# SFXiang/ORB-SLAM2-Annotation

Measured on AMD Instinct MI355X. Metric: frames/sec ORB extract+match (1000 feat, 640×480 mono) at 1/2/4/8 GPU; % HBM roofline, higher is better.
Workload: dtype u8

## Files before the change

### orb-slam2-annotation_amd/csrc/describe.hip

```cpp
#include "orbgpu_internal.h"
#include "orbgpu_kernels.h"
#include "blur_device.h"
#include "group_sum.h"
#include "../../include/orbgpu.h"

#include <algorithm>
#include <cstddef>
#include <cstdlib>
#include <type_traits>

namespace orbgpu {

namespace {

constexpr signed char kPattern[1024] = {
#include "bit_pattern_31.inc"
};
struct PatternF { float4 t[256]; };
constexpr PatternF make_pattern_f() {
    PatternF p{};
    for (int i = 0; i < 256; ++i)
        p.t[i] = float4{(float)kPattern[4 * i], (float)kPattern[4 * i + 2], (float)kPattern[4 * i + 1],
                        (float)kPattern[4 * i + 3]};
    return p;
}
__constant__ PatternF c_pattern = make_pattern_f();

constexpr int kUmax[16] = {15, 15, 15, 15, 14, 14, 14, 13, 13, 12, 11, 10, 9, 8, 6, 3};

#ifndef ORBGPU_DESC_RPITCH
#define ORBGPU_DESC_RPITCH 48
#endif
constexpr int kRPitchC = ORBGPU_DESC_RPITCH;
constexpr int kRWidth = 48;
static_assert(kRPitchC % 4 == 0 && kRPitchC >= kRWidth, "raw pitch");
constexpr int kDiscWords = 31 * 9, kDiscLoads = (kDiscWords + 63) / 64;
struct DiscWord { uint32_t m1, mc, mv, off; };
struct DiscLut { DiscWord w[4][kDiscLoads * 64]; };
constexpr DiscLut make_disc_lut() {
    DiscLut L{};
    for (int od = 0; od < 4; ++od)
        for (int idx = 0; idx < kDiscWords; ++idx) {
            const int r = idx / 9, q = idx % 9, v = r - 15, d = kUmax[v < 0 ? -v : v];
            DiscWord e{0u, 0u, 0u, (uint32_t)(r * kRPitchC + 4 * q)};
            for (int b = 0; b < 4; ++b) {
                const int u = 4 * q + b - od - 15;
                if (u >= -d && u <= d) {
                    e.m1 |= 1u << (8 * b);
                    e.mc |= (uint32_t)(4 * q + b) << (8 * b);
                    e.mv |= (uint32_t)(v + 15) << (8 * b);
                }
            }
            L.w[od][idx] = e;
        }
    return L;
}
__constant__ DiscLut c_disc = make_disc_lut();
struct DiscTail { DiscWord w[4][64]; };
constexpr DiscTail make_disc_tail() {
    DiscTail T{};
    const DiscLut L = make_disc_lut();
    for (int od = 0; od < 4; ++od)
        for (int i = 0; i < 64; ++i) T.w[od][i] = L.w[od][256 + i];
    return T;
}
__constant__ DiscTail c_disc_tail = make_disc_tail();
static_assert(kDiscLoads == 5, "the disc loads are four from c_disc and one from c_disc_tail");

__device__ inline float fast_atan2(float y, float x) {
    const float k = (float)(180 / M_PI);
    const float p1 = 0.9997878412794807f * k, p3 = -0.3258083974640975f * k;
    const float p5 = 0.1555786518463281f * k, p7 = -0.04432655554792128f * k;
    const float ax = fabsf(x), ay = fabsf(y);
    const float eps = (float)2.220446049250313080847e-16;
    float a, c, c2;
    if (ax >= ay) {
        c = __fdiv_rn(ay, __fadd_rn(ax, eps));
        c2 = __fmul_rn(c, c);
        a = __fmul_rn(__fadd_rn(__fmul_rn(__fadd_rn(__fmul_rn(__fadd_rn(__fmul_rn(p7, c2), p5), c2), p3), c2), p1), c);
    } else {
        c = __fdiv_rn(ax, __fadd_rn(ay, eps));
        c2 = __fmul_rn(c, c);
        a = __fsub_rn(90.f, __fmul_rn(__fadd_rn(__fmul_rn(__fadd_rn(__fmul_rn(__fadd_rn(__fmul_rn(p7, c2), p5), c2), p3), c2), p1), c));
    }
    if (x < 0) a = __fsub_rn(180.f, a);
    if (y < 0) a = __fsub_rn(360.f, a);
    return a;
}

struct SinCosTab { double sign[4], hpi_inv, hpi, c0, c1, c2, c3, c4, s1, s2, s3; };
__constant__ SinCosTab c_sc[2] = {
    {{1.0, -1.0, -1.0, 1.0}, 0x1.45F306DC9C883p+23, 0x1.921FB54442D18p0, 0x1p0, -0x1.ffffffd0c621cp-2,
     0x1.55553e1068f19p-5, -0x1.6c087e89a359dp-10, 0x1.99343027bf8c3p-16, -0x1.555545995a603p-3,
     0x1.1107605230bc4p-7, -0x1.994eb3774cf24p-13},
    {{1.0, -1.0, -1.0, 1.0}, 0x1.45F306DC9C883p+23, 0x1.921FB54442D18p0, -0x1p0, 0x1.ffffffd0c621cp-2,
     -0x1.55553e1068f19p-5, 0x1.6c087e89a359dp-10, -0x1.99343027bf8c3p-16, -0x1.555545995a603p-3,
     0x1.1107605230bc4p-7, -0x1.994eb3774cf24p-13}};

__device__ inline uint32_t top12(float x) { return (__float_as_uint(x) >> 20) & 0x7ff; }

__device__ inline float sc_poly(double x, double x2, const SinCosTab* p, int n) {
    if ((n & 1) == 0) {
        const double x3 = __dmul_rn(x, x2);
        const double s1 = __fma_rn(x2, p->s3, p->s2);
        const double x7 = __dmul_rn(x3, x2);
        const double s = __fma_rn(x3, p->s1, x);
        return __double2float_rn(__fma_rn(x7, s1, s));
    }
    const double x4 = __dmul_rn(x2, x2);
    const double c2 = __fma_rn(x2, p->c4, p->c3);
    const double c1 = __fma_rn(x2, p->c1, p->c0);
    const double x6 = __dmul_rn(x4, x2);
    const double c = __fma_rn(x4, p->c2, c1);
    return __double2float_rn(__fma_rn(x6, c2, c));
}

__device__ inline void glibc_sincosf(float y, float* sinp, float* cosp) {
    double x = y;
    if (top12(y) < top12(0x1.921FB6p-1f)) {
        if (top12(y) < top12(0x1p-12f)) { *sinp = y; *cosp = 1.0f; return; }
        const double x2 = __dmul_rn(x, x);
        *sinp = sc_poly(x, x2, &c_sc[0], 0);
        *cosp = sc_poly(x, x2, &c_sc[0], 1);
        return;
    }
    const double r = __dmul_rn(x, c_sc[0].hpi_inv);
    const int n = ((int32_t)r + 0x800000) >> 24;
    x = __fma_rn(-(double)n, c_sc[0].hpi, x);
    const double s = c_sc[0].sign[n & 3];
    const SinCosTab* p = (n & 2) ? &c_sc[1] : &c_sc[0];
    const double xs = __dmul_rn(x, s), x2 = __dmul_rn(x, x);
    *sinp = sc_poly(xs, x2, p, n);
    *cosp = sc_poly(xs, x2, p, n ^ 1);
}

__device__ inline uint32_t wave_total(uint32_t v) {
    v += (uint32_t)__builtin_amdgcn_update_dpp(0, (int)v, kDppXor1, 0xF, 0xF, true);
    v += (uint32_t)__builtin_amdgcn_update_dpp(0, (int)v, kDppXor2, 0xF, 0xF, true);
    v += (uint32_t)__builtin_amdgcn_update_dpp(0, (int)v, kDppHalfMirror, 0xF, 0xF, true);
    v += (uint32_t)__builtin_amdgcn_update_dpp(0, (int)v, kDppMirror, 0xF, 0xF, true);
    v += (uint32_t)__builtin_amdgcn_update_dpp(0, (int)v, 0x142, 0xA, 0xF, false);
    v += (uint32_t)__builtin_amdgcn_update_dpp(0, (int)v, 0x143, 0xC, 0xF, false);
    return (uint32_t)__builtin_amdgcn_readlane((int)v, 63);
}

constexpr int kBPitch = 40;
constexpr int kRPitch = kRPitchC;
constexpr int kRawWords = kPatch * (kRWidth / 4);
constexpr int kQuads = kBPitch / 4;
constexpr int kColChunks = (kBlur + 6) / 7;

__device__ inline void wave_sync() {
    asm volatile("s_waitcnt lgkmcnt(0)" ::: "memory");
    __builtin_amdgcn_wave_barrier();
}

__device__ inline int reflect101(int p, int n) { return p < 0 ? -p : (p >= n ? 2 * n - 2 - p : p); }

#ifndef ORBGPU_DESC_KEYS
#define ORBGPU_DESC_KEYS 1
#endif
constexpr int kKeysPerWave = ORBGPU_DESC_KEYS;

#ifndef DESC_LDS_PROBE
#define DESC_LDS_PROBE 0
#endif
static_assert(kKeysPerWave == 1 || kKeysPerWave == 2 || kKeysPerWave == 4, "ORBGPU_DESC_KEYS: 1, 2 or 4");

constexpr int kRawBytes = (kPatch * kRPitch + 15) & ~15;
constexpr int kBlurSlotBytes = (kBlur * kBPitch + 15) & ~15;
struct alignas(16) DescLds {
    uint8_t raw[kRawBytes];
    uint8_t blur[kKeysPerWave][kBlurSlotBytes];
};
static_assert(offsetof(DescLds, blur) % 16 == 0 && kBlurSlotBytes % 16 == 0, "16-byte dump stores into blur[k]");

#ifndef ORBGPU_DESC_SCALAR_COUNTS
#define ORBGPU_DESC_SCALAR_COUNTS 1
#endif

struct KeyRef {
    int l, i, before, cx, cy;
    uint32_t key;
};

__device__ bool key_ref(const Geom& g, int f, int slot, int lane, const uint32_t* __restrict__ oct_out,
                        const int* __restrict__ oct_count, int* __restrict__ counts, KeyRef& K) {
    uint32_t se = g.slot_tab[slot];
    uint32_t key = oct_out[(size_t)f * g.slots_frame + slot];
#if ORBGPU_DESC_SCALAR_COUNTS
    (void)lane;
    se = (uint32_t)__builtin_amdgcn_readfirstlane((int)se);
    key = (uint32_t)__builtin_amdgcn_readfirstlane((int)key);
    const int l = (int)(se & 15u), i = (int)(se >> 4);
    const int* cr = oct_count + (size_t)f * kOcStride;
    int cv[kMaxLevels];
#pragma unroll
    for (int j = 0; j < kMaxLevels; ++j) cv[j] = cr[j];
    int before = 0, mine = 0, total = 0;
#pragma unroll
    for (int j = 0; j < kMaxLevels; ++j) {
        const int cj = j < g.nlevels ? cv[j] : 0;
        before += j < l ? cj : 0;
        mine = j == l ? cj : mine;
        total += cj;
    }
    if (slot == 0 && lane == 0) counts[f] = total;
#else
    const int ll = lane & 15;
    int c = oct_count[(size_t)f * kOcStride + ll];
    se = (uint32_t)__builtin_amdgcn_readfirstlane((int)se);
    key = (uint32_t)__builtin_amdgcn_readfirstlane((int)key);
    asm volatile("" ::"s"(se), "s"(key), "v"(c));
    c = ll < g.nlevels ? c : 0;
    const int l = (int)(se & 15u), i = (int)(se >> 4);
    int sc = c;
    sc += __builtin_amdgcn_update_dpp(0, sc, 0x111, 0xF, 0xF, true);
    sc += __builtin_amdgcn_update_dpp(0, sc, 0x112, 0xF, 0xF, true);
    sc += __builtin_amdgcn_update_dpp(0, sc, 0x114, 0xF, 0xF, true);
    sc += __builtin_amdgcn_update_dpp(0, sc, 0x118, 0xF, 0xF, true);
    const int mine = __builtin_amdgcn_readlane(c, l);
    const int before = __builtin_amdgcn_readlane(sc, l) - mine;
    if (slot == 0 && lane == 0) counts[f] = __builtin_amdgcn_readlane(sc, 15);
#endif
    if (i >= mine) return false;
    K.l = l;
    K.i = i;
    K.before = before;
    K.key = key;
    K.cx = key_x(K.key) + kBorder;
    K.cy = key_y(K.key) + kBorder;
    return true;
}

__device__ int2 describe_patch(const Geom& g, int f, const KeyRef& K, int lane, uint8_t* rawbuf, uint8_t* blur_out,
                               const uint8_t* __restrict__ img0, size_t row0, size_t frame0,
                               const uint8_t* __restrict__ pyr) {
    const int l = K.l, cx = K.cx, cy = K.cy;
    const LevelGeom& L = g.lv[l];
#ifdef DESC_PROBE_SAMEFRAME
    const uint8_t* raw = img0;
    const size_t rp = row0;
    (void)frame0;
#else
    const uint8_t* raw = l == 0 ? img0 + (size_t)f * frame0 : pyr + L.offset + (size_t)f * L.frame_bytes;
    const size_t rp = l == 0 ? row0 : (size_t)L.pitch;
#endif

    const int xb = (cx - kBlurR) & ~3, x0 = xb - 4;
    if (x0 >= 0 && x0 + kRWidth <= L.w && cy - kPatchR >= 0 && cy + kPatchR < L.h) {
        constexpr int kChunks = kPatch * (kRWidth / 16);
        const uint8_t* top = raw + (size_t)(cy - kPatchR) * rp + x0;
        uint4 c[3];
        uint8_t* dst[3];
        uint8_t* const dump = blur_out;
#pragma unroll
        for (int k = 0; k < 3; ++k) {
            const uint32_t idx = (uint32_t)(lane + 64 * k), r = __umul24(idx, 21846u) >> 16, q = idx - 3u * r;
            const uint32_t doff = kRPitch == 48 ? 16u * idx : __umul24(r, (uint32_t)kRPitch) + 16u * q;
            dst[k] = (k < 2 && 64 * 2 <= kChunks) || idx < (uint32_t)kChunks ? rawbuf + doff : dump;
            const uint32_t idxc = k < 2 ? idx : min(idx, (uint32_t)kChunks - 1u), rc = __umul24(idxc, 21846u) >> 16;
            c[k] = load16_a4(top + (uint32_t)(__umul24(rc, (uint32_t)rp - 48u) + 16u * idxc));
        }
#pragma unroll
        for (int k = 0; k < 3; ++k) {
            if constexpr (kRPitch % 16 == 0) {
                *reinterpret_cast<uint4*>(dst[k]) = c[k];
            } else {
                uint32_t* d = reinterpret_cast<uint32_t*>(dst[k]);
                d[0] = c[k].x;
                d[1] = c[k].y;
                d[2] = c[k].z;
                d[3] = c[k].w;
            }
        }
    } else {
    constexpr int kLoads = (kRawWords + 63) / 64;
    uint32_t v[kLoads];
#pragma unroll
    for (int k = 0; k < kLoads; ++k) {
        const int idx = min(lane + 64 * k, kRawWords - 1), r = idx / 12, q = idx - r * 12;
        const uint8_t* row = raw + (size_t)reflect101(cy - kPatchR + r, L.h) * rp;
        const int col = x0 + 4 * q;
        if (col >= 0 && col + 3 < L.w) {
            v[k] = *reinterpret_cast<const uint32_t*>(row + col);
        } else {
            uint32_t w = 0;
            for (int j = 0; j < 4; ++j) w |= (uint32_t)row[reflect101(col + j, L.w)] << (8 * j);
            v[k] = w;
        }
    }
#pragma unroll
    for (int k = 0; k < kLoads; ++k) {
        const int idx = lane + 64 * k, r = idx / 12, q = idx - r * 12;
        if (idx < kRawWords) reinterpret_cast<uint32_t*>(rawbuf)[r * (kRPitch / 4) + q] = v[k];
    }
    }
    wave_sync();

    const int xd = (cx - 15) & ~3, od = cx - 15 - xd;
    const uint8_t* disc = rawbuf + (kPatchR - 15) * kRPitch + (xd - x0);
    uint32_t sp = 0u, cp = 0u, vp = 0u;
    const __attribute__((address_space(1))) uint8_t* dtab =
        (const __attribute__((address_space(1))) uint8_t*)&c_disc.w[od][0];
    const __attribute__((address_space(1))) uint8_t* dtab4 =
        (const __attribute__((address_space(1))) uint8_t*)&c_disc_tail.w[od][0];
#pragma unroll
    for (int k = 0; k < kDiscLoads; ++k) {
        typedef uint32_t u32x4 __attribute__((ext_vector_type(4)));
        const u32x4 t = *(const __attribute__((address_space(1))) u32x4*)((k < 4 ? dtab : dtab4) + 16u * (uint32_t)lane +
                                                                          1024u * (k % 4));
        const DiscWord e{t.x, t.y, t.z, t.w};
#if DESC_LDS_PROBE & 4
        const uint32_t w = *reinterpret_cast<const uint32_t*>(rawbuf + 4 * lane + 256 * k + (e.off & 0));
#else
        const uint32_t w = *reinterpret_cast<const uint32_t*>(disc + e.off);
#endif
        sp = __builtin_amdgcn_udot4(w, e.m1, sp, false);
        cp = __builtin_amdgcn_udot4(w, e.mc, cp, false);
        vp = __builtin_amdgcn_udot4(w, e.mv, vp, false);
    }
    const int m10 = (int)wave_total(cp - __umul24((uint32_t)(od + 15), sp));
    const int m01 = (int)wave_total(vp - __umul24(15u, sp));

    const int simd_end = L.w & ~3;
    auto passes = [&](auto all_simd) {
        const int qq = (int)(__umul24((uint32_t)lane, 10923u) >> 16), c = lane - qq * kColChunks;
        const int q = min(qq, kQuads - 1), r0 = c * 7;
        const bool simd = xb + 4 * q < simd_end, store = qq < kQuads;
#if DESC_LDS_PROBE & 2
        const uint32_t raw0 = 12u * (uint32_t)lane + 0u * (uint32_t)(r0 + q);
#else
        const uint32_t raw0 = __umul24((uint32_t)r0, (uint32_t)kRPitch) + 4u * (uint32_t)q;
#endif
        const uint32_t out0 = __umul24((uint32_t)r0, (uint32_t)kBPitch) + 4u * (uint32_t)q;
        auto row = [&](int k, blurdev::f32x2& lo, blurdev::f32x2& hi) {
            const uint32_t* w = reinterpret_cast<const uint32_t*>(rawbuf + raw0 + k * kRPitch);
            blurdev::Raw3 R3;
            R3.a = w[0];
            R3.b = w[1];
            R3.c = w[2];
            blurdev::row_pass_raw_shifted(R3, lo, hi);
        };
        auto from_next = [](blurdev::f32x2 v) {
            return blurdev::f32x2{
                __int_as_float(__builtin_amdgcn_mov_dpp(__float_as_int(v.x), 0x130, 0xF, 0xF, false)),
                __int_as_float(__builtin_amdgcn_mov_dpp(__float_as_int(v.y), 0x130, 0xF, 0xF, false))};
        };
        blurdev::f32x2 wl[13], wh[13];
#pragma unroll
        for (int k = 0; k < 8; ++k) row(k, wl[k], wh[k]);
#pragma unroll
        for (int j = 0; j < 7; ++j) {
            if (j >= 2) {
                wl[6 + j] = from_next(wl[j - 1]);
                wh[6 + j] = from_next(wh[j - 1]);
            }
            if (store && r0 + j < kBlur) {
                const blurdev::f32x2 lo =
                    blurdev::col_pass(wl[j], wl[j + 1], wl[j + 2], wl[j + 3], wl[j + 4], wl[j + 5], wl[j + 6]);
                const blurdev::f32x2 hi =
                    blurdev::col_pass(wh[j], wh[j + 1], wh[j + 2], wh[j + 3], wh[j + 4], wh[j + 5], wh[j + 6]);
#if DESC_LDS_PROBE & 8
                *reinterpret_cast<uint32_t*>(blur_out + ((4 * lane + 256 * j) & 1023) + (out0 & 0)) =
                    all_simd ? blurdev::pack4_simd(lo, hi) : blurdev::pack4(lo, hi, simd);
#else
                *reinterpret_cast<uint32_t*>(blur_out + out0 + j * kBPitch) =
                    all_simd ? blurdev::pack4_simd(lo, hi) : blurdev::pack4(lo, hi, simd);
#endif
            }
        }
    };
    if (xb + 4 * (kQuads - 1) < simd_end)
        passes(std::true_type{});
    else
        passes(std::false_type{});
    return int2{m10, m01};
}

__device__ void describe_tests(const Geom& g, int f, const KeyRef& K, int lane, const uint8_t* blur, float4 rot,
                               orbgpu_keypoint* __restrict__ kps, uint8_t* __restrict__ desc, int kp_cap) {
    const LevelGeom& L = g.lv[K.l];
    const int ob = K.cx - kBlurR - ((K.cx - kBlurR) & ~3);
    const float angle = rot.x, a = rot.y, b = rot.z;
    unsigned long long words[4];
    constexpr float kMagic = 12582912.f;
    constexpr uint32_t kBias = 0x400000u * (uint32_t)kBPitch + 0x4B400000u;
    const uint32_t cb = (uint32_t)(kBlurR * kBPitch + kBlurR + ob) - kBias;
    typedef float f2 __attribute__((ext_vector_type(2)));
    const f2 va = {a, a}, vb = {b, b}, vm = {kMagic, kMagic};
#pragma unroll
    for (int rnd = 0; rnd < 4; ++rnd) {
        const float4 pt = c_pattern.t[rnd * 64 + lane];
        const f2 px = {pt.x, pt.y}, py = {pt.z, pt.w};
        const f2 fy = px * vb + py * va;
        const f2 fx = px * va - py * vb;
        const f2 my = fy + vm, mx = fx + vm;
        int val[2];
#pragma unroll
        for (int pp = 0; pp < 2; ++pp) {
            const uint32_t iy = __float_as_uint(pp ? my.y : my.x), ix = __float_as_uint(pp ? mx.y : mx.x);
#if DESC_LDS_PROBE & 1
            val[pp] = blur[(int)(4u * (uint32_t)lane + (uint32_t)pp + ((__umul24(iy, (uint32_t)kBPitch) + ix + cb) & 0x300u))];
#else
            val[pp] = blur[(int)(__umul24(iy, (uint32_t)kBPitch) + ix + cb)];
#endif
        }
        words[rnd] = __ballot(val[0] < val[1]);
    }

    const size_t o = (size_t)f * kp_cap + K.before + K.i;
    if (lane == 0) {
        typedef unsigned long long u64x2 __attribute__((ext_vector_type(2)));
        auto vmov64 = [](unsigned long long x) {
            unsigned long long v;
            asm("v_mov_b64 %0, %1" : "=v"(v) : "s"(x));
            return v;
        };
        u64x2* d = reinterpret_cast<u64x2*>(desc + o * 32);
        d[0] = u64x2{vmov64(words[0]), vmov64(words[1])};
        d[1] = u64x2{vmov64(words[2]), vmov64(words[3])};
        orbgpu_keypoint kp;
        const float fx = (float)K.cx, fy = (float)K.cy;
        kp.x = K.l == 0 ? fx : __fmul_rn(fx, L.scale);
        kp.y = K.l == 0 ? fy : __fmul_rn(fy, L.scale);
        kp.size = (float)L.size_i;
        kp.angle = angle;
        kp.response = (float)key_s(K.key);
        kp.octave = K.l;
        kp.class_id = -1;
        kps[o] = kp;
    }
}

#ifdef DESC_STAMPS
__device__ unsigned long long g_desc_stamps[16];
#define DSTAMP(k) (stamp_on ? (ts[k] = __builtin_amdgcn_s_memtime()) : 0ull)
#else
#define DSTAMP(k) ((void)0)
#endif

#ifndef ORBGPU_DESC_WAVES
#define ORBGPU_DESC_WAVES 2
#endif
constexpr int kDescWaves = ORBGPU_DESC_WAVES;

__global__ __launch_bounds__(64 * kDescWaves) void describe_kernel(Geom g, int items, int f0,
                                                                   const uint8_t* __restrict__ img0, size_t row0,
                                                                   size_t frame0, const uint8_t* __restrict__ pyr,
                                                                   const uint32_t* __restrict__ oct_out,
                                                                   const int* __restrict__ oct_count,
                                                                   orbgpu_keypoint* __restrict__ kps,
                                                                   uint8_t* __restrict__ desc,
                                                                   int* __restrict__ counts, int kp_cap,
                                                                   int* __restrict__ err_word,
                                                                   int* __restrict__ err_copy) {
    __shared__ DescLds s_lds[kDescWaves];
    if (err_copy && blockIdx.x == 0 && threadIdx.x == 0) *err_copy = atomicExch(err_word, 0);
    const int lane = threadIdx.x & 63;
    const int wave = __builtin_amdgcn_readfirstlane(threadIdx.x >> 6);
#if ORBGPU_DESC_SWIZZLE
    const int blk = xcd_swizzle((int)blockIdx.x, (int)gridDim.x);
#else
    const int blk = (int)blockIdx.x;
#endif
    const int item = blk * kDescWaves + wave;
#ifdef DESC_STAMPS
    const bool stamp_on = (item & 63) == 0;
    unsigned long long ts[8] = {};
#endif
    DSTAMP(0);
    const int per_frame = (g.slots_frame + kKeysPerWave - 1) / kKeysPerWave;
    const int fi = kKeysPerWave == 1 ? (int)udiv40((uint32_t)item, g.slots_magic) : item / per_frame;
    const int slot0 = (item - fi * per_frame) * kKeysPerWave;
    const int f = f0 + fi;
    if (item >= items) return;
    KeyRef K[kKeysPerWave];
    bool valid[kKeysPerWave];
    int nvalid = 0;
#pragma unroll
    for (int k = 0; k < kKeysPerWave; ++k) {
        valid[k] = slot0 + k < g.slots_frame && key_ref(g, f, slot0 + k, lane, oct_out, oct_count, counts, K[k]);
        nvalid += valid[k];
    }
    if (nvalid == 0) return;
    DSTAMP(1);
    auto key_at = [&](int k, KeyRef& Kk) {
        int l = K[0].l, i = K[0].i, before = K[0].before, cx = K[0].cx, cy = K[0].cy;
        uint32_t key = K[0].key;
        bool v = valid[0];
#pragma unroll
        for (int j = 1; j < kKeysPerWave; ++j) {
            const bool h = k == j;
            l = h ? K[j].l : l;
            i = h ? K[j].i : i;
            before = h ? K[j].before : before;
            cx = h ? K[j].cx : cx;
            cy = h ? K[j].cy : cy;
            key = h ? K[j].key : key;
            v = h ? valid[j] : v;
        }
        Kk = KeyRef{l, i, before, cx, cy, key};
        return v;
    };
    int mx = 0, my = 0;
#pragma unroll 1
    for (int k = 0; k < kKeysPerWave; ++k) {
        KeyRef Kk;
        if (!key_at(k, Kk)) continue;
        if (k > 0) wave_sync();
        int lane_k = lane;
        asm volatile("" : "+v"(lane_k));
        const int2 mm = describe_patch(g, f, Kk, lane_k, s_lds[wave].raw, s_lds[wave].blur[k], img0, row0, frame0, pyr);
        if (kKeysPerWave == 1 || lane == k) {
            mx = mm.x;
            my = mm.y;
        }
    }
    DSTAMP(2);
    const float ang = fast_atan2((float)my, (float)mx);
    float sa, ca;
    glibc_sincosf(__fmul_rn(ang, (float)(M_PI / 180.f)), &sa, &ca);
    wave_sync();
    DSTAMP(3);
#pragma unroll 1
    for (int k = 0; k < kKeysPerWave; ++k) {
        KeyRef Kk;
        if (!key_at(k, Kk)) continue;
        const float a_k = __int_as_float(__builtin_amdgcn_readlane(__float_as_int(ang), k));
        const float c_k = __int_as_float(__builtin_amdgcn_readlane(__float_as_int(ca), k));
        const float s_k = __int_as_float(__builtin_amdgcn_readlane(__float_as_int(sa), k));
        describe_tests(g, f, Kk, lane, s_lds[wave].blur[k], float4{a_k, c_k, s_k, 0.f}, kps, desc, kp_cap);
    }
#ifdef DESC_STAMPS
    DSTAMP(4);
    if (stamp_on && lane == 0) {
        for (int k = 1; k <= 4; ++k) atomicAdd(&g_desc_stamps[k - 1], ts[k] - ts[k - 1]);
        atomicAdd(&g_desc_stamps[15], 1ull);
    }
#endif
}

}

#ifdef DESC_STAMPS
extern "C" int orbgpu_debug_desc_stamps(unsigned long long* out, int reset) {
    if (hipMemcpyFromSymbol(out, HIP_SYMBOL(g_desc_stamps), sizeof(g_desc_stamps)) != hipSuccess) return -2;
    if (reset) {
        unsigned long long z[16] = {};
        if (hipMemcpyToSymbol(HIP_SYMBOL(g_desc_stamps), z, sizeof(z)) != hipSuccess) return -2;
    }
    return 0;
}
#endif

hipError_t launch_describe(const Geom& g, int batch, const uint8_t* img0, size_t row0, size_t frame0,
                           const uint8_t* pyr, const uint32_t* oct_out, const int* oct_count,
                           orbgpu_keypoint* kps, uint8_t* desc, int* counts, int kp_cap,
                           hipStream_t stream, int* err_word, int* err_copy, int f0) {
    if (row0 >= (1u << 24)) return hipErrorInvalidValue;
    if ((size_t)g.slots_frame * batch >= (1u << 24) || g.slots_frame >= (1 << 16))
        return hipErrorInvalidValue;
    const int items = (g.slots_frame + kKeysPerWave - 1) / kKeysPerWave * batch;
    const int blocks = (items + kDescWaves - 1) / kDescWaves;
    hipLaunchKernelGGL(describe_kernel, dim3(blocks), dim3(64 * kDescWaves), 0, stream, g, items, f0, img0, row0, frame0,
                       pyr, oct_out, oct_count, kps, desc, counts, kp_cap, err_word, err_copy);
    return hipGetLastError();
}

}
```

Before: 462,900.

## Blur only the rotated-pattern footprint using a constexpr per-lane chain table

Replaces the fixed lane-to-(quad, 7-row chunk) mapping of the separable blur with a constexpr lane table. The table assigns 6-row chains only to quads and rows that the rotated BRIEF pattern can sample, built from a conservative footprint of bit_pattern_31 per sub-quad offset. Each lane loads its raw offset, output offset, row count and column from a constant LUT with one vector load. Lanes now hold 7 own rows instead of 8, so there is less LDS reading and blur arithmetic per lane. The cost is an extra constant-memory load and reliance on compile-time proofs that the footprint covers every pixel the descriptor reads.

After: 466,400, median of 6. About the same (+0.7%).

```diff
diff --git a/orb-slam2-annotation_amd/csrc/describe.hip b/orb-slam2-annotation_amd/csrc/describe.hip
--- a/orb-slam2-annotation_amd/csrc/describe.hip
+++ b/orb-slam2-annotation_amd/csrc/describe.hip
@@ -1,6 +1,7 @@
 #include "orbgpu_internal.h"
 #include "orbgpu_kernels.h"
 #include "blur_device.h"
+#include "describe_lanes.h"
 #include "group_sum.h"
 #include "../../include/orbgpu.h"
 
@@ -148,7 +149,21 @@
 constexpr int kRPitch = kRPitchC;
 constexpr int kRawWords = kPatch * (kRWidth / 4);
 constexpr int kQuads = kBPitch / 4;
-constexpr int kColChunks = (kBlur + 6) / 7;
+
+struct LaneWord { uint32_t raw0, out0, count, col; };
+struct LaneLut { LaneWord w[4][64]; };
+constexpr LaneLut make_lane_lut() {
+    static_assert(lanes::kRadius == kBlurR && lanes::kRawRows == kPatch && lanes::kQuads == kQuads, "describe_lanes.h");
+    LaneLut T{};
+    for (int ob = 0; ob < 4; ++ob)
+        for (int k = 0; k < 64; ++k) {
+            const lanes::Lane e = lanes::kLaneTable.lane[ob][k];
+            T.w[ob][k] = LaneWord{(uint32_t)(e.s * kRPitchC + 4 * e.quad), (uint32_t)(e.s * kBPitch + 4 * e.quad), e.count,
+                                  4u * e.quad};
+        }
+    return T;
+}
+__constant__ LaneLut c_lanes = make_lane_lut();
 
 __device__ inline void wave_sync() {
     asm volatile("s_waitcnt lgkmcnt(0)" ::: "memory");
@@ -305,9 +320,11 @@
         (const __attribute__((address_space(1))) uint8_t*)&c_disc.w[od][0];
     const __attribute__((address_space(1))) uint8_t* dtab4 =
         (const __attribute__((address_space(1))) uint8_t*)&c_disc_tail.w[od][0];
+    typedef uint32_t u32x4 __attribute__((ext_vector_type(4)));
+    const u32x4 lw = *(const __attribute__((address_space(1))) u32x4*)(
+        (const __attribute__((address_space(1))) uint8_t*)&c_lanes.w[cx - kBlurR - xb][0] + 16u * (uint32_t)lane);
 #pragma unroll
     for (int k = 0; k < kDiscLoads; ++k) {
-        typedef uint32_t u32x4 __attribute__((ext_vector_type(4)));
         const u32x4 t = *(const __attribute__((address_space(1))) u32x4*)((k < 4 ? dtab : dtab4) + 16u * (uint32_t)lane +
                                                                           1024u * (k % 4));
         const DiscWord e{t.x, t.y, t.z, t.w};
@@ -325,15 +342,14 @@
 
     const int simd_end = L.w & ~3;
     auto passes = [&](auto all_simd) {
-        const int qq = (int)(__umul24((uint32_t)lane, 10923u) >> 16), c = lane - qq * kColChunks;
-        const int q = min(qq, kQuads - 1), r0 = c * 7;
-        const bool simd = xb + 4 * q < simd_end, store = qq < kQuads;
+        const int count = (int)lw.z;
+        const bool simd = xb + (int)lw.w < simd_end;
 #if DESC_LDS_PROBE & 2
-        const uint32_t raw0 = 12u * (uint32_t)lane + 0u * (uint32_t)(r0 + q);
-#else
-        const uint32_t raw0 = __umul24((uint32_t)r0, (uint32_t)kRPitch) + 4u * (uint32_t)q;
-#endif
-        const uint32_t out0 = __umul24((uint32_t)r0, (uint32_t)kBPitch) + 4u * (uint32_t)q;
+        const uint32_t raw0 = 12u * (uint32_t)lane + 0u * lw.x;
+#else
+        const uint32_t raw0 = lw.x;
+#endif
+        const uint32_t out0 = lw.y;
         auto row = [&](int k, blurdev::f32x2& lo, blurdev::f32x2& hi) {
             const uint32_t* w = reinterpret_cast<const uint32_t*>(rawbuf + raw0 + k * kRPitch);
             blurdev::Raw3 R3;
@@ -347,16 +363,17 @@
                 __int_as_float(__builtin_amdgcn_mov_dpp(__float_as_int(v.x), 0x130, 0xF, 0xF, false)),
                 __int_as_float(__builtin_amdgcn_mov_dpp(__float_as_int(v.y), 0x130, 0xF, 0xF, false))};
         };
-        blurdev::f32x2 wl[13], wh[13];
-#pragma unroll
-        for (int k = 0; k < 8; ++k) row(k, wl[k], wh[k]);
-#pragma unroll
-        for (int j = 0; j < 7; ++j) {
-            if (j >= 2) {
-                wl[6 + j] = from_next(wl[j - 1]);
-                wh[6 + j] = from_next(wh[j - 1]);
+        constexpr int kOwn = lanes::kChunk + 1;
+        blurdev::f32x2 wl[kOwn + 5], wh[kOwn + 5];
+#pragma unroll
+        for (int k = 0; k < kOwn; ++k) row(k, wl[k], wh[k]);
+#pragma unroll
+        for (int j = 0; j < lanes::kChunk; ++j) {
+            if (j >= 1) {
+                wl[6 + j] = from_next(wl[j]);
+                wh[6 + j] = from_next(wh[j]);
             }
-            if (store && r0 + j < kBlur) {
+            if (j < count) {
                 const blurdev::f32x2 lo =
                     blurdev::col_pass(wl[j], wl[j + 1], wl[j + 2], wl[j + 3], wl[j + 4], wl[j + 5], wl[j + 6]);
                 const blurdev::f32x2 hi =
diff --git a/orb-slam2-annotation_amd/csrc/describe_lanes.h b/orb-slam2-annotation_amd/csrc/describe_lanes.h
--- /dev/null
+++ b/orb-slam2-annotation_amd/csrc/describe_lanes.h
@@ -0,0 +1,150 @@
+#pragma once
+
+#include <stdint.h>
+
+namespace orbgpu {
+namespace lanes {
+
+constexpr int kRadius = 18;
+constexpr int kRows = 2 * kRadius + 1;
+constexpr int kRawRows = kRows + 6;
+constexpr int kQuads = 10;
+constexpr int kChunk = 6;
+constexpr int kLanes = 64;
+
+constexpr signed char kPattern[1024] = {
+#include "bit_pattern_31.inc"
+};
+
+constexpr double csqrt(double v) {
+    if (v <= 0.0) return 0.0;
+    double x = v < 1.0 ? 1.0 : v;
+    for (int i = 0; i < 64; ++i) {
+        const double n = 0.5 * (x + v / x);
+        if (n == x) break;
+        x = n;
+    }
+    return x;
+}
+
+struct Footprint {
+    bool in[2 * kRadius * kRadius + 1];
+    constexpr bool at(int x, int y) const { return in[x * x + y * y]; }
+};
+constexpr Footprint make_footprint() {
+    constexpr int kMaxR2 = 2 * 13 * 13;
+    constexpr double kTol = 0.70710678118654752440 + 0.01;
+    int below[kMaxR2 + 2] = {};
+    bool has[kMaxR2 + 1] = {};
+    for (int i = 0; i < 512; ++i) has[kPattern[2 * i] * kPattern[2 * i] + kPattern[2 * i + 1] * kPattern[2 * i + 1]] = true;
+    for (int v = 0; v <= kMaxR2; ++v) below[v + 1] = below[v] + (has[v] ? 1 : 0);
+    Footprint F{};
+    for (int d2 = 0; d2 <= 2 * kRadius * kRadius; ++d2) {
+        const double d = csqrt((double)d2), lo = d > kTol ? (d - kTol) * (d - kTol) : 0.0, hi = (d + kTol) * (d + kTol);
+        int a = (int)lo, b = (int)hi;
+        if ((double)a < lo) ++a;
+        if (b > kMaxR2) b = kMaxR2;
+        F.in[d2] = a <= b && below[b + 1] - below[a] > 0;
+    }
+    return F;
+}
+constexpr Footprint kFootprint = make_footprint();
+
+struct Lane {
+    uint8_t quad, s, count;
+};
+struct Quad {
+    uint8_t first, last;
+};
+struct LaneTable {
+    Lane lane[4][kLanes];
+    Quad quad[4][kQuads];
+    int used[4];
+};
+
+constexpr LaneTable make_lane_table() {
+    LaneTable T{};
+    for (int ob = 0; ob < 4; ++ob) {
+        int n = 0;
+        for (int q = 0; q < kQuads; ++q) {
+            int first = kRows, last = -1;
+            for (int j = 0; j < kRows; ++j)
+                for (int b = 0; b < 4; ++b) {
+                    const int x = 4 * q + b - kRadius - ob;
+                    if (x < -kRadius || x > kRadius || !kFootprint.at(x, j - kRadius)) continue;
+                    if (j < first) first = j;
+                    last = j;
+                }
+            T.quad[ob][q] = Quad{(uint8_t)first, (uint8_t)(last < 0 ? 0 : last)};
+            if (last < 0) continue;
+            const int rows = last - first + 1, len = (rows + kChunk - 1 + kChunk - 1) / kChunk;
+            const int span = kChunk * (len - 1);
+            int s0 = first - (span + 1 - rows) / 2;
+            if (s0 + span > kRows - 1) s0 = kRows - 1 - span;
+            if (s0 < 0) s0 = 0;
+            for (int k = 0; k < len; ++k, ++n)
+                if (n < kLanes) T.lane[ob][n] = Lane{(uint8_t)q, (uint8_t)(s0 + kChunk * k), (uint8_t)(k + 1 < len ? kChunk : 1)};
+        }
+        T.used[ob] = n;
+        for (int k = n; k < kLanes; ++k) T.lane[ob][k] = Lane{T.lane[ob][0].quad, T.lane[ob][0].s, 0};
+    }
+    return T;
+}
+constexpr LaneTable kLaneTable = make_lane_table();
+
+constexpr int footprint_pixels() {
+    int n = 0;
+    for (int y = -kRadius; y <= kRadius; ++y)
+        for (int x = -kRadius; x <= kRadius; ++x) n += kFootprint.at(x, y) ? 1 : 0;
+    return n;
+}
+constexpr bool lanes_fit() {
+    for (int ob = 0; ob < 4; ++ob)
+        if (kLaneTable.used[ob] > kLanes) return false;
+    return true;
+}
+constexpr bool rows_inside() {
+    for (int ob = 0; ob < 4; ++ob)
+        for (int k = 0; k < kLanes; ++k) {
+            const Lane e = kLaneTable.lane[ob][k];
+            if (e.quad >= kQuads || e.s + 6 > kRawRows - 1 || e.count > kChunk || e.s + e.count > kRows) return false;
+        }
+    return true;
+}
+constexpr bool chains_adjacent() {
+    for (int ob = 0; ob < 4; ++ob)
+        for (int k = 0; k < kLanes; ++k) {
+            const Lane e = kLaneTable.lane[ob][k];
+            if (e.count <= 1) continue;
+            if (k + 1 >= kLanes) return false;
+            const Lane nx = kLaneTable.lane[ob][k + 1];
+            if (nx.quad != e.quad || nx.s != e.s + kChunk) return false;
+        }
+    return true;
+}
+constexpr bool footprint_covered() {
+    for (int ob = 0; ob < 4; ++ob) {
+        int writers[kQuads][kRows] = {};
+        for (int k = 0; k < kLanes; ++k) {
+            const Lane e = kLaneTable.lane[ob][k];
+            for (int j = 0; j < e.count; ++j) ++writers[e.quad][e.s + j];
+        }
+        for (int q = 0; q < kQuads; ++q)
+            for (int j = 0; j < kRows; ++j) {
+                if (writers[q][j] > 1) return false;
+                for (int b = 0; b < 4; ++b) {
+                    const int x = 4 * q + b - kRadius - ob;
+                    if (x >= -kRadius && x <= kRadius && kFootprint.at(x, j - kRadius) && writers[q][j] != 1) return false;
+                }
+            }
+    }
+    return true;
+}
+static_assert(footprint_pixels() == 1124, "the footprint of bit_pattern_31.inc");
+static_assert(lanes_fit(), "at most 64 chain lanes per ob");
+static_assert(rows_inside(), "owned rows within raw rows 0..42, stored rows within 0..36");
+static_assert(chains_adjacent(), "a chain's lanes are consecutive, 6 rows apart");
+static_assert(footprint_covered(), "every footprint pixel is computed, once, for every ob");
+
+}
+}
```
